# massquantity/tdfo

Measured on AMD Instinct MI355X. Metric: examples/sec (whole node) DLRM on Criteo-1TB-shaped synthetic, higher is better.
Workload: dtype bf16; 1 GPU; model=DLRM, global_batch=8192, parallelism=single-gpu, tables=criteo-1tb, embedding_dim=128, per_gpu_batch=8192

## Files before the change

### csrc/bindings.cpp

```cpp
#include <cmath>
#include <cstring>

#include <ATen/ATen.h>
#include <ATen/hip/HIPContext.h>
#include <torch/library.h>

#include "tdfo_kernels.h"

namespace {

using at::Tensor;

hipStream_t cur_stream() { return at::hip::getCurrentHIPStream().stream(); }

const uint16_t* bf16_ptr(const Tensor& t) {
  TORCH_CHECK(t.scalar_type() == at::kBFloat16, "expected bf16 tensor");
  return reinterpret_cast<const uint16_t*>(t.data_ptr());
}
uint16_t* bf16_mut(const Tensor& t) {
  TORCH_CHECK(t.scalar_type() == at::kBFloat16, "expected bf16 tensor");
  return reinterpret_cast<uint16_t*>(t.data_ptr());
}
void check_dev(const Tensor& t, const char* name) {
  TORCH_CHECK(t.is_cuda(), name, " must be a GPU tensor");
// ... 1087 lines not shown
  const float* bp[3] = {nullptr, nullptr, nullptr};
  int64_t bst[3] = {0, 0, 0};
  for (int i = 0; i < 3; ++i) {
    if (*bs[i]) {
      const Tensor& b = **bs[i];
      check_dev(b, "bias");
      TORCH_CHECK(b.scalar_type() == at::kFloat && b.dim() == 1 && b.size(0) >= nout[i],
                  "bottom_mlp_fwd: bias fp32 1-D");
      bp[i] = b.data_ptr<float>();
      bst[i] = b.stride(0);
    }
  }
  a.b0 = bp[0]; a.b1 = bp[1]; a.b2 = bp[2]; a.bs0 = bst[0]; a.bs1 = bst[1]; a.bs2 = bst[2];
  a.y0 = bf16_mut(y0); a.y1 = bf16_mut(y1); a.y2 = bf16_mut(y2);
  a.ldy0 = y0.stride(0); a.ldy1 = y1.stride(0); a.ldy2 = y2.stride(0);
  a.M = (int)M;
  if (dense) {
    check_dev(*dense, "dense");
    TORCH_CHECK(dense->scalar_type() == at::kFloat && dense->dim() == 2 && dense->size(0) == M &&
                dense->stride(1) == 1 && dense->size(1) <= 16 && dense->size(1) < x.size(1),
                "bottom_mlp_fwd: dense fp32 [M, nd < 16] rows");
    a.dense = dense->data_ptr<float>(); a.ld_dense = dense->stride(0);
    a.nd = (int)dense->size(1);
    a.x_out = bf16_mut(x);
    if (label_src) {
      TORCH_CHECK(label_dst && label_src->scalar_type() == at::kFloat &&
                  label_dst->scalar_type() == at::kFloat && label_src->is_contiguous() &&
                  label_dst->is_contiguous() && label_src->numel() >= M &&
                  label_dst->numel() >= M, "bottom_mlp_fwd: labels fp32 [M]");
      a.label_src = label_src->data_ptr<float>(); a.label_dst = label_dst->data_ptr<float>();
    }
  }
  tdfo::bottom_mlp_fwd(a, cur_stream());
}

void check_bf16_buf(const Tensor& t, int64_t n, const char* name) {
  check_dev(t, name);
  TORCH_CHECK(t.scalar_type() == at::kBFloat16 && t.is_contiguous() && t.numel() >= n, name,
              ": bf16 contiguous buffer too small");
}

void rw_rows_gather(const Tensor& Wt, const Tensor& recv, int64_t W, int64_t cap, const Tensor& out) {
  check_dev(Wt, "W");
  TORCH_CHECK(Wt.scalar_type() == at::kFloat && Wt.is_contiguous() && Wt.dim() == 2, "W fp32 2-D");
  TORCH_CHECK(Wt.size(0) <= (1LL << 32), "rw: owner rows must fit 32-bit row keys");
  const int64_t D = Wt.size(1);
  TORCH_CHECK(D == 16 || D == 32 || D == 64 || D == 128 || D == 256, "rw_rows_gather: D unsupported");
  check_i64(recv, "recv");
  TORCH_CHECK(recv.numel() == W * (cap + 1), "rw recv buffer must be [W][cap+1]");
  check_bf16_buf(out, W * (cap + 1) * D, "rw rows out");
  tdfo::rw_rows_gather(Wt.data_ptr<float>(), (int)D, recv.data_ptr<int64_t>(), (int)W, cap,
                       bf16_mut(out), cur_stream());
}

void rw_rows_scatter(const Tensor& send, int64_t W, int64_t cap, int64_t B, int64_t D,
                     const Tensor& rows, const Tensor& region, int64_t ld, const Tensor& map,
                     int64_t nrw) {
  check_i64(send, "send");
  TORCH_CHECK(send.numel() == W * (cap + 1), "rw send buffer must be [W][cap+1]");
  TORCH_CHECK(D == 16 || D == 32 || D == 64 || D == 128 || D == 256, "rw_rows_scatter: D unsupported");
  TORCH_CHECK(ld >= nrw * D && ld % 4 == 0, "rw_rows_scatter: row stride");
  TORCH_CHECK(B * ld < (1LL << 31), "rw_rows_scatter: region offsets must fit int32");
  check_bf16_buf(rows, W * (cap + 1) * D, "rw rows");
  check_bf16_buf(region, B * ld, "rw pooled region");
  check_dev(map, "rw map");
  TORCH_CHECK(map.scalar_type() == at::kInt && map.numel() >= W * (cap + 1), "rw map int32 [W][cap+1]");
// ... 873 lines not shown
  m.def("embedding_bwd(Tensor(a!) W, Tensor row_offset, Tensor indices, Tensor offsets, Tensor grad_off, "
        "Tensor? psw, int T, int B, bool mean, int key_bits, Tensor grad, int grad_stride, int opt, "
        "Tensor(b!)? state1, Tensor(c!)? state2, Tensor hyper, float eps, float beta1, float beta2, "
        "float weight_decay, Tensor(d!)? dense_grad, int segsort, int sr_seed=0, "
        "Tensor(e!)? sr_counter=None, bool sr=False) -> ()");
  m.def("embedding_bwd_workspace(int nnz, int D) -> int", [](int64_t nnz, int64_t D) {
    return (int64_t)tdfo::embedding_bwd_workspace(nnz < 1 ? 1 : nnz, (int)D);
  });
  m.def("embedding_bwd_prepare(Tensor W, Tensor row_offset, Tensor indices, Tensor offsets, "
        "Tensor grad_off, Tensor? psw, int T, int B, bool mean, int key_bits, int grad_stride, "
        "int segsort, Tensor(a!) workspace, Tensor? bag_len=None, Tensor(b!)? sr_counter=None) -> ()");
  m.def("embedding_bwd_apply(Tensor(a!) W, Tensor row_offset, Tensor indices, Tensor offsets, "
        "Tensor grad_off, Tensor? psw, int T, int B, bool mean, int key_bits, Tensor grad, "
        "int grad_stride, int opt, Tensor(b!)? state1, Tensor(c!)? state2, Tensor hyper, "
        "float eps, float beta1, float beta2, float weight_decay, Tensor(d!)? dense_grad, "
        "int segsort, Tensor(e!) workspace, int sr_seed=0, Tensor? sr_counter=None, "
        "bool sr=False) -> ()");
  m.def("embedding_dense_update(Tensor(a!) W, Tensor(d!) grad, int rows, int opt, Tensor(b!)? state1, "
        "Tensor(c!)? state2, Tensor hyper, float eps, float beta1, float beta2, "
        "float weight_decay, bool clear_grad) -> ()");
  m.def("rw_bucketize_workspace(int n, int W) -> int", rw_bucketize_workspace);
  m.def("rw_bucketize(Tensor ids, Tensor meta, int nrw, int W, int B, int cap, int n, "
        "Tensor(a!) send, Tensor(b!) workspace, Tensor(c!) overflow) -> ()");
  m.def("rw_pool(Tensor Wt, Tensor recv, Tensor meta, int nrw, int W, int B, int cap, bool mean, "
        "Tensor(a!) starts, Tensor(b!) out, int out_ld) -> ()");
  m.def("embedding_bwd_prepare_rw(Tensor W, Tensor recv, Tensor meta, int nrw, int Wsz, int B, "
        "int cap, bool mean, int key_bits, int grad_ld, int dummy_row, Tensor(a!) workspace, "
        "int rows=0) -> ()");
  m.def("rw_rows_gather(Tensor Wt, Tensor recv, int W, int cap, Tensor(a!) out) -> ()");
  m.def("bottom_mlp_fwd_ok(int k0, int n0, int n1, int n2) -> bool", bottom_mlp_fwd_ok);
  m.def("bottom_mlp_fwd(Tensor x, Tensor w0, Tensor w1, Tensor w2, Tensor? b0, Tensor? b1, "
        "Tensor? b2, Tensor(a!) y0, Tensor(b!) y1, Tensor(c!) y2, Tensor? dense, Tensor? label_src, "
        "Tensor(d!)? label_dst) -> ()");
  m.def("rw_rows_scatter(Tensor send, int W, int cap, int B, int D, Tensor rows, Tensor(a!) region, "
        "int ld, Tensor(b!) map, int nrw) -> ()");
  m.def("rw_grads_gather(Tensor map, int W, int cap, int D, Tensor dregion, Tensor(a!) gsend) -> ()");
  m.def("embedding_bwd_apply_rw(Tensor(a!) W, int Wsz, int B, int cap, bool mean, int key_bits, "
        "Tensor grad, int opt, Tensor(b!)? state1, Tensor(c!)? state2, Tensor hyper, float eps, "
        "float beta1, float beta2, float weight_decay, Tensor(d!) workspace) -> ()");
  m.def("dense_optimizer(Tensor(a!) p, Tensor g, Tensor(b!)? m, Tensor(c!)? v, Tensor(d!)? p_bf16, int opt, "
        "Tensor hyper, float beta1, float beta2, float eps, float wd, float momentum, Tensor? found_inf, "
        "Tensor[] seg_slabs, int[] seg_start, int[] seg_splits) -> ()");
  m.def("check_finite(Tensor g, Tensor(a!) found) -> ()");
  m.def("sort_pairs(Tensor keys, Tensor vals, int key_bits) -> (Tensor, Tensor)");
  m.def("cast_bf16(Tensor x, Tensor(a!) y) -> ()");
  m.def("bf16_stochastic_round(Tensor x, int seed, Tensor counter, int row0, Tensor(a!) out) -> ()");
  m.def("synth_criteo(int seed, int rank, int batch_index, int B, Tensor rows, Tensor pooling, "
        "Tensor base, int dist, float alpha, Tensor w_dense, Tensor table_bias, Tensor(a!) dense, "
        "Tensor(b!) ids, Tensor(c!) label) -> ()");
  m.def("synth_ids(int seed, int rank, int index_base, int B, Tensor rows, Tensor pooling, "
        "Tensor base, int dist, float alpha, Tensor counter, int nnz, Tensor(a!) ids) -> ()");
  m.def("synth_dense(int seed, int rank, int index_base, int B, Tensor rows, Tensor pooling, "
        "Tensor base, int dist, float alpha, Tensor counter, Tensor w_dense, Tensor table_bias, "
        "Tensor(a!) x0, Tensor(b!) label) -> ()");
  m.def("batch_load(Tensor dense, Tensor(a!) x0, Tensor ids, Tensor(b!) ids_dst, Tensor label, "
        "Tensor(c!) label_dst) -> ()");
  m.def("head_bce(Tensor H, Tensor w, Tensor b, Tensor label, float inv_n, bool relu_mask, "
        "Tensor(a!) logits, Tensor(b!) dH, Tensor(c!) part) -> ()");
  m.def("head_reduce(Tensor part, int nparts, int K, Tensor(a!) grad, Tensor(b!) loss_acc, "
        "Tensor(c!)[] bumps, bool defer) -> ()");
  m.def("reduce_rows(Tensor inp, int rows, int n, int ld, Tensor(a!) out, bool accumulate, float scale) -> ()");
  m.def("colsum(Tensor x, Tensor(a!) out, bool accumulate) -> ()");
  m.def("slab_reduce(Tensor[] slabs, int[] splits, Tensor(a!)[] outs) -> ()");
  m.def("seg_copy(Tensor src, Tensor(a!) dst, Tensor chunks, int src_n, int dst_n) -> ()");
  m.def("piece_copy(Tensor(a!) buf, Tensor pieces, int B, int w, int extent) -> ()");
  m.def("auc_hist(Tensor logits, Tensor labels, int nb, Tensor(a!) hist) -> ()");
// ... 23 lines not shown

TORCH_LIBRARY_IMPL(tdfo, CUDA, m) {
  m.impl("gemm", gemm);
  m.impl("attention_fwd", attention_fwd);
  m.impl("encoder_layer_fwd", encoder_layer_fwd);
  m.impl("encoder_layer_bwd", encoder_layer_bwd);
  m.impl("attention_bwd", attention_bwd);
  m.impl("attention_stream_fwd", attention_stream_fwd);
  m.impl("attention_stream_bwd", attention_stream_bwd);
  m.impl("layernorm_fwd", layernorm_fwd);
  m.impl("layernorm_bwd", layernorm_bwd);
  m.impl("seq_prologue_fwd", seq_prologue_fwd);
  m.impl("rank_metrics", rank_metrics);
  m.impl("topk_scores", topk_scores);
  m.impl("seq_prologue_bwd", seq_prologue_bwd);
  m.impl("gather_columns", gather_columns);
  m.impl("concat_features", concat_features);
  m.impl("batch_load", batch_load);
  m.impl("synth_criteo", synth_criteo);
  m.impl("split_features", split_features);
  m.impl("cross_bwd", cross_bwd);
  m.impl("interaction_fwd", interaction_fwd);
  m.impl("interaction_bwd", interaction_bwd);
  m.impl("embedding_bag_fwd", embedding_bag_fwd);
  m.impl("embedding_bwd", embedding_bwd);
  m.impl("embedding_bwd_prepare", embedding_bwd_prepare);
  m.impl("embedding_bwd_apply", embedding_bwd_apply);
  m.impl("embedding_dense_update", embedding_dense_update);
  m.impl("rw_bucketize", rw_bucketize);
  m.impl("rw_pool", rw_pool);
  m.impl("embedding_bwd_prepare_rw", embedding_bwd_prepare_rw);
  m.impl("rw_rows_gather", rw_rows_gather);
  m.impl("bottom_mlp_fwd", bottom_mlp_fwd);
  m.impl("rw_rows_scatter", rw_rows_scatter);
  m.impl("rw_grads_gather", rw_grads_gather);
  m.impl("embedding_bwd_apply_rw", embedding_bwd_apply_rw);
  m.impl("dense_optimizer", dense_optimizer);
  m.impl("check_finite", check_finite);
  m.impl("sort_pairs", sort_pairs);
  m.impl("cast_bf16", cast_bf16);
  m.impl("bf16_stochastic_round", bf16_stochastic_round);
  m.impl("slab_reduce", slab_reduce);
  m.impl("synth_ids", synth_ids);
  m.impl("synth_dense", synth_dense);
  m.impl("seg_copy", seg_copy);
  m.impl("piece_copy", piece_copy);
  m.impl("head_bce", head_bce);
  m.impl("reduce_rows", reduce_rows);
  m.impl("head_reduce", head_reduce);
  m.impl("colsum", colsum);
  m.impl("auc_hist", auc_hist);
  m.impl("two_tower", two_tower);
  m.impl("reduce_adam", reduce_adam);
  m.impl("linear_xent", linear_xent);
  m.impl("linear_xent_rows", linear_xent_rows);
  m.impl("linear_bce_rows", linear_bce_rows);
  m.impl("sample_ids", sample_ids);
  m.impl("jagged_to_dense", jagged_to_dense);
  m.impl("dense_to_jagged", dense_to_jagged);
  m.impl("jagged_ids_to_dense", jagged_ids_to_dense);
}

TORCH_LIBRARY_IMPL(tdfo, CPU, m) {
  m.impl("auc_hist", auc_hist);
}
```

### csrc/include/tdfo_kernels.h

```cpp
#pragma once
#include <hip/hip_runtime.h>
#include <stdint.h>

namespace tdfo {

struct GemmArgs {
  const uint16_t* A; int64_t lda; int a_col;
  const uint16_t* B; int64_t ldb; int b_col;
  int M, N, K, splits;
  const float* bias; int64_t bias_stride;
  int relu;
  const uint16_t* mask; int64_t ldm;
  uint16_t* C; int64_t ldc;
  float* C32; int64_t ldc32;
  const uint16_t* mul; int64_t ldmul;
  const uint16_t* add; int64_t ldadd;
  uint16_t* C2; int64_t ldc2;
  int csum_on, csum_col;
};
void gemm_bf16(const GemmArgs& a, hipStream_t s);


void gemm_group(const GemmArgs* a, int n, hipStream_t s);
int gemm_pairing(int v);
// ... 116 lines not shown

void embedding_dense_update(const EmbBwdArgs& a, int64_t rows, const float* grad, float* clear,
                            hipStream_t s);

struct SynthArgs {
  uint64_t seed; int rank; int64_t batch_index;
  int B, num_dense, T;
  const int64_t* rows; const int* pooling; const int64_t* base;
  int dist; double alpha;
  const float* w_dense; const float* table_bias;
  float* dense; int64_t* ids; float* label;
  const float* index_ptr; uint16_t* x0; int64_t ldx;
};
void synth_criteo(const SynthArgs& a, hipStream_t s);
void synth_ids(const SynthArgs& a, hipStream_t s);
void synth_dense(const SynthArgs& a, hipStream_t s);

struct BotMlpArgs {
  const uint16_t* x; int64_t ldx;
  const uint16_t* w0; const uint16_t* w1; const uint16_t* w2;
  int64_t ldw0, ldw1, ldw2;
  const float* b0; const float* b1; const float* b2;
  int64_t bs0, bs1, bs2;
  uint16_t* y0; uint16_t* y1; uint16_t* y2;
  int64_t ldy0, ldy1, ldy2;
  int M;
  const float* dense = nullptr; int64_t ld_dense = 0; int nd = 0;
  uint16_t* x_out = nullptr;
  const float* label_src = nullptr; float* label_dst = nullptr;
};
bool bottom_mlp_fwd_supported(int k0, int n0, int n1, int n2);
void bottom_mlp_fwd(const BotMlpArgs& a, hipStream_t s);

struct RwBucketArgs {
  const int64_t* ids; const int64_t* meta;
  int nrw, W, B; int64_t cap; int64_t n;
  int64_t* send; int32_t* overflow; int32_t* need;
};
size_t rw_bucketize_workspace(int64_t n, int W);
void rw_bucketize(const RwBucketArgs& a, void* ws, hipStream_t s);
struct RwPoolArgs {
  const float* Wt; int D; const int64_t* recv; const int64_t* meta;
  int nrw, W, B; int64_t cap; int mean;
  int32_t* starts; void* out; int out_f32; int64_t out_ld;
};
void rw_pool(const RwPoolArgs& a, hipStream_t s);
void rw_rows_gather(const float* Wt, int D, const int64_t* recv, int W, int64_t cap,
                    uint16_t* out, hipStream_t s);
void rw_rows_scatter(const int64_t* send, int W, int64_t cap, int B, int D, const uint16_t* rows,
                     uint16_t* region, int64_t ld, int32_t* map, hipStream_t s);
void rw_grads_gather(const int32_t* map, int W, int64_t cap, int D, const uint16_t* dregion,
                     uint16_t* gsend, hipStream_t s);
void embedding_bwd_prepare_rw(const EmbBwdArgs& a, const int64_t* recv, const int64_t* meta,
                              int nrw, int W, int64_t cap, int64_t grad_ld, int64_t dummy_row,
                              int rows, hipStream_t s);

enum DenseOpt { OPT_ADAMW = 0, OPT_ADAM = 1, OPT_SGD = 2, OPT_ADAGRAD = 3 };
struct DenseOptArgs {
  float* p; const float* g; float* m; float* v; uint16_t* p_bf16;
  int64_t n; int opt;
  const float* hyper;
  float beta1, beta2, eps, weight_decay, momentum;
  const float* found_inf;
  int nseg;
  int64_t seg_start[16], seg_len[16];
  int seg_splits[16];
// ... 216 lines not shown
```

### tdfo_amd/models/dlrm.py

```python
from __future__ import annotations

import math
import os
import warnings
from dataclasses import dataclass, field
from typing import List, Optional, Sequence

import torch

from ..utils.capture import graph_capture
from .. import ops
from .dlrm_dcn import DCNMixin
from .dlrm_streams import StreamGraphsMixin
from .dlrm_multirank import MultiRankStreamsMixin
from ..parallel.comm import as_comm, dense_comm_for
from ..sparse.planner import ShardingPlan, plan_sharding
from ..sparse.sharded import ShardedEmbeddingBags
from ..sparse.tables import EmbOptimConfig, TableConfig
from ..utils.flat import FlatParams

CRITEO_1TB_ROWS = [39884406, 39043, 17289, 7420, 20263, 3, 7120, 1543, 63, 38532951, 2953546,
                   403346, 10, 2208, 11938, 155, 4, 976, 14, 39979771, 25641295, 39664984, 585935,
                   12972, 108, 36]
CRITEO_KAGGLE_ROWS = [1460, 583, 10131227, 2202608, 305, 24, 12517, 633, 3, 93145, 5683, 8351593,
# ... 198 lines not shown
        opt = DENSE_OPTS[cfg.dense_opt]
        self.dense_opt = opt
        fp.finalize(dev, with_adam=opt in (ops.OPT_ADAMW, ops.OPT_ADAM))
        self.fp = fp
        self._ar_split = fp.offset(self.top_layers[0].name + ".w")
        self._init_dense()
        if world_size > 1:
            self.comm.broadcast(fp.p, src=0)
        fp.sync_bf16()
        self._defer_top_wgrad = (world_size > 1 if cfg.defer_wgrad is None
                                 else bool(cfg.defer_wgrad))
        bf = torch.bfloat16

        def z(*shape, dt=bf):
            return torch.zeros(*shape, dtype=dt, device=dev)

        def act_in(L: Lin):
            t = z(B, L.wcols)
            t[:, L.bcol] = 1.0
            return t

        self.x0 = act_in(self.bottom_layers[0])
        self.bot_in = [self.x0] + [act_in(L) for L in self.bottom_layers[1:]]
        self.h_out = z(B, D)
        Lb = self.bottom_layers
        self._fused_bottom = (
            dev.type == "cuda" and len(Lb) == 3 and D == Lb[2].out
            and os.environ.get("TDFO_FUSED_BOTTOM", "1") != "0"
            and Lb[0].in_k == Lb[0].wcols and not Lb[1].bias_in_k and not Lb[2].bias_in_k
            and Lb[1].in_k == Lb[0].out and Lb[2].in_k == Lb[1].out
            and ops.bottom_mlp_fwd_ok(Lb[0].in_k, Lb[0].out, Lb[1].out, Lb[2].out))
        self._bot_load_fold = os.environ.get("TDFO_BOT_LOAD_FOLD", "1") != "0"
        self._head_side = os.environ.get("TDFO_HEAD_SIDE", "1") != "0"
        self.bot_grad = [z(B, L.out) for L in self.bottom_layers]
        self.top_in = [act_in(L) for L in self.top_layers]
        self.t_out = z(B, self.head_k)
        self.top_grad = [z(B, L.out) for L in self.top_layers]
        self.dz = z(B, self.top_layers[0].in_k)
        self.label = z(B, dt=torch.float32)
        self.ids = torch.zeros(self.emb.nnz_local, dtype=torch.int64, device=dev)
        self.emb.bind_ids(self.ids)
        if cfg.interaction == "dcn":
            Lc, Wd, r = cfg.dcn_layers, self.top_real, cfg.dcn_rank
            self.dcn_x = [z(B, Wd) for _ in range(Lc)] + [self.top_in[0]]
            self.dcn_h = [act_in(u) for u in self.dcn_u]
            self.dcn_y = [z(B, Wd) for _ in range(Lc)]
            self.dcn_dx = [z(B, Wd) for _ in range(Lc + 1)]
            self.dcn_dx0acc = z(B, Wd)
            nb = Lc if self._defer_top_wgrad else 1
            self.dcn_dhl = [z(B, r) for _ in range(nb)]
            self.dcn_dyl = [z(B, Wd) for _ in range(nb)]
        self._x0_alias = False
        if (cfg.interaction == "dcn" and not self._defer_top_wgrad
                and self.emb.alias_pooled(self.dcn_x[0], self.dcn_dx[0], D)):
            self._x0_alias = True
            self.h_out = self.dcn_x[0][:, :D]
        self.logits = z(B, dt=torch.float32)
        self.nparts = ops.head_parts(B)
        self.head_part = z(self.nparts * (self.head_k + 2), dt=torch.float32)
        self.loss_sum = z(1, dt=torch.float32)
        self._pair_bwd = dev.type == "cuda"
        dcn = cfg.interaction == "dcn"
        if dev.type == "cuda" and not os.environ.get("TDFO_GEMM_POLICY"):
            ops.gemm_policy(5 if dcn else 0)
        self._gemm_pol = ops.gemm_policy(-1) if dev.type == "cuda" else None
        self._csum = not (dcn and dev.type == "cuda" and ops.gemm_policy(-1) in (4, 5))
# ... 133 lines not shown
        self._next = (dense, ids, label)
        self._primed = True
        self._mr_inflight = True

    def set_next_batch(self, dense: torch.Tensor, ids: torch.Tensor, label: torch.Tensor):
        if self.graph == "mstreams":
            self._mr_stage_next(dense, ids, label)
            return
        self._next = (dense, ids, label)

    def _m_load_next(self):
        if self._whole_capture:
            sx, si, sl = self._stg
            self.x0.copy_(sx)
            self.ids.copy_(si)
            self.label.copy_(sl)
            return
        dense, ids, label = self._next
        ops.batch_load(dense, self.x0, ids, self.ids, label, self.label)

    def _m_ids_exchange_next(self):
        self.emb.stage_fwd_ids_exchange(async_op=True, lagged=self._rw_lagged)

    def _rw_resolve(self):
        if self._rw_lagged and self.emb.rw_resolve_need():
            self.sync_streams()
            self.emb.rw_redo()

    def _fwd(self, L: Lin, x, out, relu=True):
        W = self.fp.bf16(L.name + ".w")
        bias = None if L.bias_in_k else self.fp.param(L.name + ".w")[:, L.bcol]
        ops.gemm(x[:, :L.in_k], False, W[:, :L.in_k], False, bias, relu, None, out, None, 1)

    def _bwd(self, L: Lin, x, dy, dx, x_is_relu, wgrad_now: bool = True):
        if not wgrad_now:
            self._dgrad(L, x, dy, dx, x_is_relu)
            return
        with ops.gemm_batch(self._pair_bwd and dx is not None):
            self._wgrad_gemm(L, x, dy)
            self._dgrad(L, x, dy, dx, x_is_relu)

    def _wg_splits(self, M: int, N: int) -> int:
        return ops.wgrad_splits(M, N, self.B, 256, slots=self._wg_slots)

    def _wgrad_n(self, L: Lin) -> int:
        return L.in_k if self._csum else L.wcols

    def _wgrad(self, L: Lin, x, dy):
        self._wgrad_gemm(L, x, dy)

    def _wgrad_gemm(self, L: Lin, x, dy):
        csum = -1 if (L.bias_in_k or not self._csum) else L.bcol
        n = self._wgrad_n(L)
        g = self.fp.grad(L.name + ".w").view(-1)
        if L.name in self.wslab:
            sl, S = self.wslab[L.name]
            ops.gemm(dy, True, x[:, :n], True, None, False, None, None, sl, S,
                     ldc32=L.wcols, csum_col=csum)
        else:
            ops.gemm(dy, True, x[:, :n], True, None, False, None, None, g, 1,
                     ldc32=L.wcols, csum_col=csum)
        return None

    def _dgrad(self, L: Lin, x, dy, dx, x_is_relu):
        if dx is not None:
            n = min(dx.shape[1], L.in_k)
            W = self.fp.bf16(L.name + ".w")
            ops.gemm(dy, False, W[:, :n], True, None, False,
                     x[:, :n] if x_is_relu else None, dx[:, :n], None, 1)

    def _stages(self):
# ... 129 lines not shown
        if self._pipe_lookup and self._ev_lookup is not None and self._side() is not None:
            torch.cuda.current_stream().wait_event(self._ev_lookup)
        self.emb.forward_wait()

    def _m_mark_loaded(self):
        if self._ev_loaded is not None and not self._whole_capture:
            self._ev_loaded.record(torch.cuda.current_stream())

    def _m_out_exchange_next(self):
        self.emb.stage_fwd_out_exchange()
        if self._ev_lookup is not None and not self._whole_capture:
            self._ev_lookup.record(torch.cuda.current_stream())

    def _s_top(self):
        self._s_top_a()
        self._s_top_b()

    def _s_top_a(self):
        cfg, fp, B = self.cfg, self.fp, self.B
        D, F = cfg.embedding_dim, self.F
        emb = self.emb
        if self._ps is not None and not self._mstream:
            self._wait(self._ps, torch.cuda.current_stream())
            with torch.cuda.stream(self._ps):
                emb.stage_bwd_prepare()
        h = self.h_out
        L0 = self.top_layers[0]
        if cfg.interaction == "dot":
            ops.interaction_fwd(h, emb.recv, self.slot_off, self.slot_stride, F, D, self.top_in[0],
                                L0.bcol)
        else:
            self._dcn_forward(h)
        n = len(self.top_layers)
        for i, L in enumerate(self.top_layers):
            out = self.top_in[i + 1][:, :L.out] if i + 1 < n else self.t_out
            self._fwd(L, self.top_in[i], out)
        K = self.head_k
        head = fp.param("head")
        ops.head_bce(self.t_out, head[:K], head[K:], self.label, 1.0 / (B * self.world), True,
                     self.logits, self.top_grad[-1], self.head_part)
        defer = self._head_side and self.device.type == "cuda"
        ops.head_reduce(self.head_part, self.nparts, K, fp.grad("head"), self.loss_sum,
                        (self.dense_hyper, self.emb_hyper), defer=defer)
        for i in reversed(range(n)):
            L = self.top_layers[i]
            if i > 0:
                dx = self.top_grad[i - 1]
            else:
                dx = self.dz if cfg.interaction == "dot" else self.dcn_dx[-1]
            self._bwd(L, self.top_in[i], self.top_grad[i], dx, x_is_relu=i > 0,
                      wgrad_now=not self._defer_top_wgrad)
            if defer:
                ops.flush_side_job()

    def _s_top_b(self):
        cfg = self.cfg
        D, F = cfg.embedding_dim, self.F
        emb = self.emb
        h = self.h_out
        if cfg.interaction == "dot":
            ops.interaction_bwd(self.dz, h, emb.recv, self.slot_off, self.slot_stride, F, D,
                                self.bot_grad[-1], emb.d_recv, self.slot_off, self.slot_stride,
                                True)
        else:
            self._dcn_backward(h)
        if not self._whole_capture:
            emb.stage_bwd_local(self.emb_hyper)
        if not self._mstream and self._ps is not None:
            self._wait(torch.cuda.current_stream(), self._ps)

    def _s_top_wgrad(self):
        if self._defer_top_wgrad:
            with ops.gemm_batch(self._pair_bwd):
                for i in reversed(range(len(self.top_layers))):
                    self._wgrad_gemm(self.top_layers[i], self.top_in[i], self.top_grad[i])
                for i in reversed(range(len(self.dcn_u))):
                    dy, _ = self._dcn_bufs(i)
                    self._wgrad_gemm(self.dcn_u[i], self.dcn_h[i], dy)
            for i in reversed(range(len(self.dcn_u))):
                self._dcn_wgrad_v(i)

    def _s_bottom_bwd(self):
        for i in reversed(range(len(self.bottom_layers))):
            L = self.bottom_layers[i]
            dx = self.bot_grad[i - 1] if i > 0 else None
            self._bwd(L, self.bot_in[i], self.bot_grad[i], dx, x_is_relu=i > 0)

    def _reduce_slabs(self, lo: int, hi: int):
        mine = [(sl, S, g) for off, sl, S, g in self._slab_sums if lo <= off < hi]
        if mine:
            ops.slab_reduce(mine)

    def _ar_issue(self, lo: int, hi: int):
        self._reduce_slabs(lo, hi)
        g = self.fp.g[lo:hi]
        if self.cfg.dense_comm == "bf16":
            if getattr(self, "_g16", None) is None:
                self._g16 = torch.empty(self.fp.g.numel(), dtype=torch.bfloat16,
                                        device=self.device)
            b = self._g16[lo:hi]
            ops.cast_bf16(g, b)
            return (self.dcomm.all_reduce(b, async_op=True), g, b)
        return (self.dcomm.all_reduce(g, async_op=True), None, None)

    def _m_allreduce_top_start(self):
        self._ar_top = None
        if self.world > 1:
            self._ar_top = self._ar_issue(self._ar_split, self.fp.g.numel())

    def _m_allreduce_start(self):
        self._ar_work = None
        if self.world > 1:
            self._ar_work = self._ar_issue(0, self._ar_split)

    def _s_emb_update(self):
        self.emb.stage_bwd_update(self.emb_hyper)

    def _m_allreduce_wait(self, names=("_ar_top", "_ar_work")):
# ... 232 lines not shown
```

### tdfo_amd/ops/__init__.py

```python
from __future__ import annotations

import os

import torch

from . import reference as ref
from ._ext import available as native_available
from ._ext import ops as _native
from .reference import (EMB_ADAGRAD, EMB_ADAM, EMB_DENSE_GRAD, EMB_ROWWISE_ADAGRAD,
                        EMB_SGD, OPT_ADAGRAD, OPT_ADAM, OPT_ADAMW, OPT_SGD, key_bits_for)


def _gpu(t: torch.Tensor) -> bool:
    return t.is_cuda


def bottom_mlp_fwd_ok(k0: int, n0: int, n1: int, n2: int) -> bool:
    return bool(native_available() and _native().bottom_mlp_fwd_ok(int(k0), int(n0), int(n1),
                                                                    int(n2)))


def bottom_mlp_fwd(x, w0, w1, w2, b0, b1, b2, y0, y1, y2, dense=None, label=None):
    ls, ld = label if label is not None else (None, None)
    _native().bottom_mlp_fwd(x, w0, w1, w2, b0, b1, b2, y0, y1, y2, dense, ls, ld)
# ... 369 lines not shown

def dense_optimizer(p, g, m, v, p_bf16, opt, hyper, beta1=0.9, beta2=0.999, eps=1e-8, wd=0.0,
                    momentum=0.0, found_inf=None, segments=()):
    if _gpu(p):
        _native().dense_optimizer(p, g, m, v, p_bf16, opt, hyper, beta1, beta2, eps, wd, momentum,
                                  found_inf, [s[1] for s in segments],
                                  [int(s[0]) for s in segments], [int(s[2]) for s in segments])
    else:
        if segments:
            g = g.clone()
            for start, slab, splits in segments:
                n = slab.numel() // splits
                g[start:start + n] = slab.view(splits, n).sum(0)
        ref.dense_optimizer(p, g, m, v, p_bf16, opt, hyper, beta1, beta2, eps, wd, momentum,
                            found_inf)


def check_finite(g, found):
    if _gpu(g):
        _native().check_finite(g, found)
    else:
        ref.check_finite(g, found)


def head_parts(B: int) -> int:
    return (B + 15) // 16


def head_bce(H, w, b, label, inv_n, relu_mask, logits, dH, part):
    if _gpu(H):
        _native().head_bce(H, w, b, label, inv_n, relu_mask, logits, dH, part)
    else:
        ref.head_bce(H, w, b, label, inv_n, relu_mask, logits, dH, part)


def reduce_rows(inp, rows, n, ld, out, accumulate=False, scale=1.0):
    if _gpu(inp):
        _native().reduce_rows(inp, rows, n, ld, out, accumulate, scale)
    else:
        ref.reduce_rows(inp, rows, n, ld, out, accumulate, scale)


class SegmentMap:

    CHUNK = 4096

    def __init__(self, pieces, device):
        self.device = torch.device(device)
        pieces = [(int(a), int(b), int(n)) for a, b, n in pieces if int(n) > 0]
        self.src_n = max([a + n for a, _, n in pieces], default=0)
        self.dst_n = max([b + n for _, b, n in pieces], default=0)
        self.n = sum(n for _, _, n in pieces)
        if self.device.type == "cuda":
            ch = []
            for a, b, n in pieces:
                for o in range(0, n, self.CHUNK):
                    ch.append((a + o, b + o, min(self.CHUNK, n - o)))
            self.chunks = torch.tensor(ch if ch else [[0, 0, 0]], dtype=torch.int64,
                                       device=self.device).view(-1, 3)
            self.nchunks = len(ch)
        else:
            idx = torch.zeros(self.dst_n, dtype=torch.int64)
            for a, b, n in pieces:
                idx[b:b + n] = torch.arange(a, a + n)
            self.index = idx

# ... 495 lines not shown
```

Measured before the change: 20.11 million examples/s.

## Fuse last top-MLP layer forward, BCE head, and dgrad into one kernel

Adds a fused HIP kernel that computes the last top-MLP layer (512->256 GEMM with bias+ReLU), the BCE head (logits, loss partials, head gradient), and the layer's input gradient (dgrad with ReLU mask) in one launch, keeping the activation tile in LDS. This removes separate GEMM, head_bce and dgrad launches and the HBM round trips of the intermediate activations. The layer's weight gradient is paired with the next layer's backward GEMM batch, or optionally with the bottom MLP. Cost: heavy LDS use limits occupancy, and the kernel only supports fixed dimensions.

```diff
diff --git a/csrc/bindings.cpp b/csrc/bindings.cpp
--- a/csrc/bindings.cpp
+++ b/csrc/bindings.cpp
@@ -1143,6 +1143,50 @@
     }
   }
   tdfo::bottom_mlp_fwd(a, cur_stream());
+}
+
+bool top_tail_ok(int64_t k, int64_t n, int64_t head_k) {
+  return tdfo::top_tail_supported((int)k, (int)n, (int)head_k);
+}
+
+void top_tail(const Tensor& x, const Tensor& w, const Tensor& bias, const Tensor& t,
+              const Tensor& hw, const Tensor& hb, const Tensor& label, double inv_n,
+              const Tensor& logits, const Tensor& dt, const Tensor& part, const Tensor& dx) {
+  TORCH_CHECK(!g_gemm_batch.on, "top_tail inside ops.gemm_batch");
+  const Tensor* ts[5] = {&x, &w, &t, &dt, &dx};
+  const char* nm[5] = {"x", "w", "t", "dt", "dx"};
+  for (int i = 0; i < 5; ++i) {
+    check_dev(*ts[i], nm[i]);
+    TORCH_CHECK(ts[i]->scalar_type() == at::kBFloat16 && ts[i]->dim() == 2 &&
+                ts[i]->stride(1) == 1 && ts[i]->stride(0) % 8 == 0 && aligned16(ts[i]->data_ptr()),
+                "top_tail: ", nm[i], " must be bf16 2-D, unit column stride, 16-B rows");
+  }
+  const int64_t B = x.size(0), K = x.size(1), N = w.size(0);
+  TORCH_CHECK(B >= 1 && B < (1LL << 31), "top_tail: batch");
+  TORCH_CHECK(tdfo::top_tail_supported((int)K, (int)N, (int)hw.numel()) && w.size(1) == K,
+              "top_tail: unsupported dims");
+  TORCH_CHECK(t.size(0) == B && t.size(1) == N && dt.size(0) == B && dt.size(1) == N &&
+              dx.size(0) == B && dx.size(1) == K, "top_tail: output shapes");
+  check_dev(bias, "bias");
+  TORCH_CHECK(bias.scalar_type() == at::kFloat && bias.dim() == 1 && bias.size(0) == N,
+              "top_tail: bias fp32 [N]");
+  check_f32c(hw, "head w"); check_f32c(hb, "head b"); check_f32c(label, "label");
+  check_f32c(logits, "logits"); check_f32c(part, "part");
+  TORCH_CHECK(hb.numel() == 1 && label.numel() == B && logits.numel() == B, "top_tail: head shapes");
+  TORCH_CHECK(part.numel() >= tdfo::head_bce_parts((int)B) * (N + 2), "top_tail: part too small");
+  tdfo::TopTailArgs a{};
+  a.x = bf16_ptr(x); a.ldx = x.stride(0);
+  a.w = bf16_ptr(w); a.ldw = w.stride(0);
+  a.bias = bias.data_ptr<float>(); a.bs = bias.stride(0);
+  a.t = bf16_mut(t); a.ldt = t.stride(0);
+  a.hw = hw.data_ptr<float>(); a.hb = hb.data_ptr<float>();
+  a.label = label.data_ptr<float>(); a.inv_n = (float)inv_n;
+  a.logits = logits.data_ptr<float>();
+  a.dt = bf16_mut(dt); a.lddt = dt.stride(0);
+  a.part = part.data_ptr<float>();
+  a.dx = bf16_mut(dx); a.lddx = dx.stride(0);
+  a.B = (int)B;
+  tdfo::top_tail(a, cur_stream());
 }
 
 void check_bf16_buf(const Tensor& t, int64_t n, const char* name) {
@@ -2082,6 +2126,10 @@
   m.def("bottom_mlp_fwd(Tensor x, Tensor w0, Tensor w1, Tensor w2, Tensor? b0, Tensor? b1, "
         "Tensor? b2, Tensor(a!) y0, Tensor(b!) y1, Tensor(c!) y2, Tensor? dense, Tensor? label_src, "
         "Tensor(d!)? label_dst) -> ()");
+  m.def("top_tail_ok(int k, int n, int head_k) -> bool", top_tail_ok);
+  m.def("top_tail(Tensor x, Tensor w, Tensor bias, Tensor(a!) t, Tensor hw, Tensor hb, "
+        "Tensor label, float inv_n, Tensor(b!) logits, Tensor(c!) dt, Tensor(d!) part, "
+        "Tensor(e!) dx) -> ()");
   m.def("rw_rows_scatter(Tensor send, int W, int cap, int B, int D, Tensor rows, Tensor(a!) region, "
         "int ld, Tensor(b!) map, int nrw) -> ()");
   m.def("rw_grads_gather(Tensor map, int W, int cap, int D, Tensor dregion, Tensor(a!) gsend) -> ()");
@@ -2171,6 +2219,7 @@
   m.impl("embedding_bwd_prepare_rw", embedding_bwd_prepare_rw);
   m.impl("rw_rows_gather", rw_rows_gather);
   m.impl("bottom_mlp_fwd", bottom_mlp_fwd);
+  m.impl("top_tail", top_tail);
   m.impl("rw_rows_scatter", rw_rows_scatter);
   m.impl("rw_grads_gather", rw_grads_gather);
   m.impl("embedding_bwd_apply_rw", embedding_bwd_apply_rw);
diff --git a/csrc/include/tdfo_kernels.h b/csrc/include/tdfo_kernels.h
--- a/csrc/include/tdfo_kernels.h
+++ b/csrc/include/tdfo_kernels.h
@@ -172,6 +172,22 @@
 bool bottom_mlp_fwd_supported(int k0, int n0, int n1, int n2);
 void bottom_mlp_fwd(const BotMlpArgs& a, hipStream_t s);
 
+struct TopTailArgs {
+  const uint16_t* x; int64_t ldx;
+  const uint16_t* w; int64_t ldw;
+  const float* bias; int64_t bs;
+  uint16_t* t; int64_t ldt;
+  const float* hw; const float* hb;
+  const float* label; float inv_n;
+  float* logits;
+  uint16_t* dt; int64_t lddt;
+  float* part;
+  uint16_t* dx; int64_t lddx;
+  int B;
+};
+bool top_tail_supported(int k, int n, int head_k);
+void top_tail(const TopTailArgs& a, hipStream_t s);
+
 struct RwBucketArgs {
   const int64_t* ids; const int64_t* meta;
   int nrw, W, B; int64_t cap; int64_t n;
diff --git a/csrc/kernels/top_tail.hip b/csrc/kernels/top_tail.hip
--- /dev/null
+++ b/csrc/kernels/top_tail.hip
@@ -0,0 +1,331 @@
+#include "tdfo_common.h"
+#include "tdfo_kernels.h"
+
+namespace tdfo {
+namespace {
+
+typedef __attribute__((ext_vector_type(4))) uint32_t u32x4;
+typedef __attribute__((ext_vector_type(2))) uint32_t u32x2;
+typedef __attribute__((address_space(1))) const void* gptr_t;
+
+constexpr int TM = 32, KX = 512, NT = 256, HK = 256;
+constexpr int SLOT = 64 * 1024;
+constexpr int R_W = 0, R_X = SLOT, R_T = 2 * SLOT, R_RED = R_T + TM * NT * 2;
+constexpr int RED_LD = HK + 2;
+constexpr int TAIL_LDS = R_RED + 2 * 4 * RED_LD * 4;
+static_assert(TAIL_LDS <= 160 * 1024, "LDS per workgroup");
+
+__device__ __forceinline__ int swz(int r, int c) { return r * 128 + ((c ^ (r & 7)) << 4); }
+
+__device__ __forceinline__ bf16x8_t frag(const TDFO_LDS char* img, int r0, int ks, int lane) {
+  const int r = r0 + (lane & 15);
+  return *(const TDFO_LDS bf16x8_t*)(img + swz(r, ks * 4 + (lane >> 4)));
+}
+
+__device__ __forceinline__ int t_off(int m, int n) {
+  return (n >> 6) * (TM * 128) + swz(m, (n & 63) >> 3) + (n & 7) * 2;
+}
+
+__device__ __forceinline__ bf16x8_t gfrag(const uint16_t* W, int64_t ldw, int r0, int kb,
+                                          int lane) {
+  const u32x4 v = *(const u32x4*)(W + (int64_t)(r0 + (lane & 15)) * ldw + kb + 8 * (lane >> 4));
+  return __builtin_bit_cast(bf16x8_t, v);
+}
+
+__device__ __forceinline__ int swz_col(int k) {
+  return ((k & 3) | (((k >> 3) & 1) << 2)) << 1;
+}
+
+__device__ __forceinline__ void glds16_asm(const void* src, TDFO_LDS char* dst) {
+  const uint32_t lds = __builtin_amdgcn_readfirstlane((uint32_t)(uintptr_t)dst);
+  asm volatile("s_mov_b32 m0, %1\n\tglobal_load_lds_dwordx4 %0, off"
+               :: "v"(src), "s"(lds) : "memory", "m0");
+}
+
+constexpr int W_PIECES = 16;
+
+__device__ __forceinline__ void stage_w(const uint16_t* W, int64_t ldw, int kt,
+                                        TDFO_LDS char* slot, int w, int lane) {
+  TDFO_LDS char* img = slot + w * (64 * 256);
+#pragma unroll
+  for (int ii = 0; ii < W_PIECES; ++ii) {
+    const int kr = ii * 4 + (lane >> 4);
+    const int c = (lane & 15) ^ swz_col(kr);
+    glds16_asm(W + (int64_t)(kt * 64 + kr) * ldw + w * 128 + c * 8, img + ii * 1024);
+  }
+}
+
+__device__ __forceinline__ bf16x8_t frag_col(const TDFO_LDS char* tile, int c0, int ks,
+                                             int lane) {
+  const int i = lane & 15, g = lane >> 4;
+  const int q = i >> 2, p = i & 3;
+  const int m = c0 + 4 * p;
+  s16x4_t v[2];
+#pragma unroll
+  for (int h = 0; h < 2; ++h) {
+    const int k = ks * 32 + 8 * g + 4 * h + q;
+    const int off = k * 256 + (((m >> 3) ^ swz_col(k)) << 4) + ((m & 7) << 1);
+    v[h] = __builtin_amdgcn_ds_read_tr16_b64_v4i16((TDFO_LDS s16x4_t*)(tile + off));
+  }
+  s16x8_t r = {v[0][0], v[0][1], v[0][2], v[0][3], v[1][0], v[1][1], v[1][2], v[1][3]};
+  return __builtin_bit_cast(bf16x8_t, r);
+}
+
+__device__ __forceinline__ void lds_wait() { asm volatile("s_waitcnt lgkmcnt(0)" ::: "memory"); }
+
+__device__ __forceinline__ void raw_barrier() {
+  __builtin_amdgcn_sched_barrier(0);
+  __builtin_amdgcn_s_barrier();
+  asm volatile("" ::: "memory");
+  __builtin_amdgcn_sched_barrier(0);
+}
+
+__device__ __forceinline__ float head_sample(const float (&hv)[4], const float (&wr)[4],
+                                             float hbias, float y, float inv_n, bool lane0,
+                                             float& x, float (&dw)[4], float& db, float& lsum) {
+#pragma clang fp contract(off)
+  float d = 0.f;
+#pragma unroll
+  for (int u = 0; u < 4; ++u) d = __builtin_fmaf(hv[u], wr[u], d);
+  x = wave_sum(d) + hbias;
+  const float sig = 1.f / (1.f + __expf(-x));
+  const float g = (sig - y) * inv_n;
+  if (lane0) {
+    lsum += __builtin_fmaf(-y, x, fmaxf(x, 0.f)) + log1pf(__expf(-fabsf(x)));
+    db += g;
+  }
+#pragma unroll
+  for (int u = 0; u < 4; ++u) dw[u] = __builtin_fmaf(g, hv[u], dw[u]);
+  return g;
+}
+
+__global__ __launch_bounds__(256) void top_tail_kernel(TopTailArgs a) {
+  extern __shared__ __attribute__((aligned(16))) char smem_raw[];
+  TDFO_LDS char* sm = (TDFO_LDS char*)smem_raw;
+  const int tid = threadIdx.x, lane = tid & 63;
+  const int w = __builtin_amdgcn_readfirstlane(tid >> 6);
+  const int m0 = blockIdx.x * TM;
+  const int B = a.B;
+
+  constexpr int J = NT / 64, S = KX / 32, PD = 8;
+  const int c0 = w * (NT / 4);
+  u32x4 xv[KX / 64];
+  {
+    const int r = tid >> 3, c = tid & 7;
+    int gr = m0 + r;
+    gr = gr < B ? gr : B - 1;
+#pragma unroll
+    for (int kt = 0; kt < KX / 64; ++kt)
+      xv[kt] = *(const u32x4*)(a.x + (int64_t)gr * a.ldx + kt * 64 + c * 8);
+  }
+  bf16x8_t b[S][J];
+#pragma unroll
+  for (int s = 0; s < PD; ++s)
+#pragma unroll
+    for (int j = 0; j < J; ++j) b[s][j] = gfrag(a.w, a.ldw, c0 + 16 * j, 32 * s, lane);
+  float bv[J][4];
+#pragma unroll
+  for (int j = 0; j < J; ++j)
+#pragma unroll
+    for (int r = 0; r < 4; ++r)
+      bv[j][r] = a.bias[(int64_t)(c0 + 16 * j + 4 * (lane >> 4) + r) * a.bs];
+  const int e0 = lane * 4;
+  float wr[4];
+#pragma unroll
+  for (int u = 0; u < 4; ++u) wr[u] = a.hw[e0 + u];
+  const float hbias = a.hb[0];
+  float yv[2][4];
+#pragma unroll
+  for (int g = 0; g < 2; ++g)
+#pragma unroll
+    for (int q = 0; q < 4; ++q) yv[g][q] = a.label[min(m0 + 16 * g + w + 4 * q, B - 1)];
+  {
+    const int r = tid >> 3, c = tid & 7;
+#pragma unroll
+    for (int kt = 0; kt < KX / 64; ++kt)
+      *(TDFO_LDS u32x4*)(sm + R_X + kt * (TM * 128) + swz(r, c)) = xv[kt];
+  }
+  __syncthreads();
+  {
+    f32x4_t acc[2][J];
+#pragma unroll
+    for (int i = 0; i < 2; ++i)
+#pragma unroll
+      for (int j = 0; j < J; ++j) acc[i][j] = (f32x4_t){0.f, 0.f, 0.f, 0.f};
+#pragma unroll
+    for (int s = 0; s < S; ++s) {
+      if (s + PD < S) {
+#pragma unroll
+        for (int j = 0; j < J; ++j)
+          b[s + PD][j] = gfrag(a.w, a.ldw, c0 + 16 * j, 32 * (s + PD), lane);
+      }
+      bf16x8_t af[2];
+#pragma unroll
+      for (int i = 0; i < 2; ++i)
+        af[i] = frag(sm + R_X + (s >> 1) * (TM * 128), 16 * i, s & 1, lane);
+#pragma unroll
+      for (int i = 0; i < 2; ++i)
+#pragma unroll
+        for (int j = 0; j < J; ++j)
+          acc[i][j] = __builtin_amdgcn_mfma_f32_16x16x32_bf16(b[s][j], af[i], acc[i][j], 0, 0, 0);
+    }
+    stage_w(a.w, a.ldw, 0, sm + R_W, w, lane);
+#pragma unroll
+    for (int j = 0; j < J; ++j) {
+      const int n = c0 + 16 * j + 4 * (lane >> 4);
+#pragma unroll
+      for (int i = 0; i < 2; ++i) {
+        const int m = 16 * i + (lane & 15);
+        float v[4];
+#pragma unroll
+        for (int r = 0; r < 4; ++r) v[r] = fmaxf(acc[i][j][r] + bv[j][r], 0.f);
+        const u32x2 pk = {pack2bf(v[0], v[1]), pack2bf(v[2], v[3])};
+        if (m0 + m < B) *(u32x2*)(a.t + (int64_t)(m0 + m) * a.ldt + n) = pk;
+        *(TDFO_LDS u32x2*)(sm + R_T + t_off(m, n)) = pk;
+      }
+    }
+  }
+  __syncthreads();
+  stage_w(a.w, a.ldw, 1, sm + R_X, w, lane);
+
+  float* red = (float*)(smem_raw + R_RED);
+#pragma unroll
+  for (int g = 0; g < 2; ++g) {
+    const int s0 = m0 + 16 * g;
+    float dw[4] = {0.f, 0.f, 0.f, 0.f};
+    float db = 0.f, lsum = 0.f;
+    float hv[4][4];
+#pragma unroll
+    for (int q = 0; q < 4; ++q) {
+      const u32x2 tv = *(const TDFO_LDS u32x2*)(sm + R_T + t_off(16 * g + w + 4 * q, e0));
+      hv[q][0] = bf2f((uint16_t)(tv.x & 0xffff));
+      hv[q][1] = bf2f((uint16_t)(tv.x >> 16));
+      hv[q][2] = bf2f((uint16_t)(tv.y & 0xffff));
+      hv[q][3] = bf2f((uint16_t)(tv.y >> 16));
+    }
+#pragma unroll
+    for (int q = 0; q < 4; ++q) {
+      const int s = s0 + w + 4 * q;
+      if (s >= B) break;
+      float x;
+      const float gq = head_sample(hv[q], wr, hbias, yv[g][q], a.inv_n, lane == 0, x, dw, db, lsum);
+      if (lane == 0) a.logits[s] = x;
+      uint16_t hb16[4];
+#pragma unroll
+      for (int u = 0; u < 4; ++u) {
+        float gh = gq * wr[u];
+        if (!(hv[q][u] > 0.f)) gh = 0.f;
+        hb16[u] = f2bf(gh);
+      }
+      const u32x2 pk = {(uint32_t)hb16[0] | ((uint32_t)hb16[1] << 16),
+                        (uint32_t)hb16[2] | ((uint32_t)hb16[3] << 16)};
+      *(u32x2*)(a.dt + (int64_t)s * a.lddt + e0) = pk;
+      *(TDFO_LDS u32x2*)(sm + R_T + t_off(16 * g + w + 4 * q, e0)) = pk;
+    }
+    float* rw = red + (g * 4 + w) * RED_LD;
+#pragma unroll
+    for (int u = 0; u < 4; ++u) rw[e0 + u] = dw[u];
+    if (lane == 0) { rw[HK] = db; rw[HK + 1] = lsum; }
+  }
+  __syncthreads();
+#pragma unroll
+  for (int g = 0; g < 2; ++g) {
+    if (m0 + 16 * g < B) {
+      const float* rg = red + g * 4 * RED_LD;
+      for (int j = tid; j < RED_LD; j += 256)
+        a.part[(int64_t)(blockIdx.x * 2 + g) * RED_LD + j] =
+            rg[j] + rg[RED_LD + j] + rg[2 * RED_LD + j] + rg[3 * RED_LD + j];
+    }
+  }
+
+  constexpr int NJ = 8;
+  const TDFO_LDS char* wimg0 = sm + R_W + w * (64 * 256);
+  const TDFO_LDS char* wimg1 = sm + R_X + w * (64 * 256);
+  f32x4_t acc[2][NJ];
+#pragma unroll
+  for (int i = 0; i < 2; ++i)
+#pragma unroll
+    for (int j = 0; j < NJ; ++j) acc[i][j] = (f32x4_t){0.f, 0.f, 0.f, 0.f};
+  auto tile = [&](int kt, const TDFO_LDS char* wimg) {
+#pragma unroll
+    for (int ks = 0; ks < 2; ++ks) {
+      bf16x8_t af[2], bfr[NJ];
+#pragma unroll
+      for (int j = 0; j < NJ; ++j) bfr[j] = frag_col(wimg, 16 * j, ks, lane);
+#pragma unroll
+      for (int i = 0; i < 2; ++i) af[i] = frag(sm + R_T + kt * (TM * 128), 16 * i, ks, lane);
+#pragma unroll
+      for (int i = 0; i < 2; ++i)
+#pragma unroll
+        for (int j = 0; j < NJ; ++j)
+          acc[i][j] = __builtin_amdgcn_mfma_f32_16x16x32_bf16(bfr[j], af[i], acc[i][j], 0, 0, 0);
+    }
+  };
+  asm volatile("s_waitcnt vmcnt(0) lgkmcnt(0)" ::: "memory");
+  raw_barrier();
+  tile(0, wimg0);
+  lds_wait();
+  raw_barrier();
+  stage_w(a.w, a.ldw, 2, sm + R_W, w, lane);
+  tile(1, wimg1);
+  lds_wait();
+  raw_barrier();
+  stage_w(a.w, a.ldw, 3, sm + R_X, w, lane);
+  asm volatile("s_waitcnt vmcnt(%0)" :: "i"(W_PIECES) : "memory");
+  raw_barrier();
+  const int rho = lane & 15, gq = lane >> 4;
+  const int mrow = (gq & 1) * 16 + rho;
+  const int ncol = w * 128 + 8 * (gq >> 1);
+  u32x4 mk[NJ];
+  {
+    int gr = m0 + mrow;
+    gr = gr < B ? gr : B - 1;
+#pragma unroll
+    for (int j = 0; j < NJ; ++j)
+      mk[j] = *(const u32x4*)(a.x + (int64_t)gr * a.ldx + ncol + 16 * j);
+  }
+  tile(2, wimg0);
+  asm volatile("s_waitcnt vmcnt(0)" ::: "memory");
+  raw_barrier();
+  tile(3, wimg1);
+#pragma unroll
+  for (int j = 0; j < NJ; ++j) {
+    float v[8];
+#pragma unroll
+    for (int r = 0; r < 4; ++r) {
+      const float p = acc[0][j][r] + 0.f, q = acc[1][j][r] + 0.f;
+      const auto sw = __builtin_amdgcn_permlane16_swap(__float_as_uint(p), __float_as_uint(q),
+                                                       false, false);
+      v[r] = __uint_as_float(sw[0]);
+      v[4 + r] = __uint_as_float(sw[1]);
+    }
+    const uint32_t mu[4] = {mk[j].x, mk[j].y, mk[j].z, mk[j].w};
+#pragma unroll
+    for (int q = 0; q < 4; ++q) {
+      if (!(bf2f((uint16_t)(mu[q] & 0xffff)) > 0.f)) v[2 * q] = 0.f;
+      if (!(bf2f((uint16_t)(mu[q] >> 16)) > 0.f)) v[2 * q + 1] = 0.f;
+    }
+    if (m0 + mrow < B)
+      *(u32x4*)(a.dx + (int64_t)(m0 + mrow) * a.lddx + ncol + 16 * j) =
+          u32x4{pack2bf(v[0], v[1]), pack2bf(v[2], v[3]), pack2bf(v[4], v[5]),
+                pack2bf(v[6], v[7])};
+  }
+}
+
+}
+
+bool top_tail_supported(int k, int n, int head_k) { return k == KX && n == NT && head_k == HK; }
+
+void top_tail(const TopTailArgs& a, hipStream_t s) {
+  if (a.B <= 0) return;
+  static bool attr = false;
+  if (!attr) {
+    TDFO_CHECK_HIP(hipFuncSetAttribute((const void*)top_tail_kernel,
+                                       hipFuncAttributeMaxDynamicSharedMemorySize, TAIL_LDS));
+    attr = true;
+  }
+  hipLaunchKernelGGL(top_tail_kernel, dim3((a.B + TM - 1) / TM), dim3(256), TAIL_LDS, s, a);
+  TDFO_CHECK_HIP(hipGetLastError());
+}
+
+}
diff --git a/tdfo_amd/models/dlrm.py b/tdfo_amd/models/dlrm.py
--- a/tdfo_amd/models/dlrm.py
+++ b/tdfo_amd/models/dlrm.py
@@ -254,6 +254,15 @@
             and ops.bottom_mlp_fwd_ok(Lb[0].in_k, Lb[0].out, Lb[1].out, Lb[2].out))
         self._bot_load_fold = os.environ.get("TDFO_BOT_LOAD_FOLD", "1") != "0"
         self._head_side = os.environ.get("TDFO_HEAD_SIDE", "1") != "0"
+        Lt = self.top_layers
+        self._top_tail = (
+            dev.type == "cuda" and len(Lt) >= 2 and not Lt[-1].bias_in_k
+            and Lt[-1].in_k == Lt[-2].out
+            and os.environ.get("TDFO_TOP_TAIL", "1") != "0"
+            and ops.top_tail_ok(Lt[-1].in_k, Lt[-1].out, self.head_k))
+        self._tail_wgrad_late = (world_size == 1 and not self._defer_top_wgrad
+                                 and cfg.opt_placement == "one_pass"
+                                 and os.environ.get("TDFO_TAIL_WGRAD", "top") == "bottom")
         self.bot_grad = [z(B, L.out) for L in self.bottom_layers]
         self.top_in = [act_in(L) for L in self.top_layers]
         self.t_out = z(B, self.head_k)
@@ -453,11 +462,13 @@
         bias = None if L.bias_in_k else self.fp.param(L.name + ".w")[:, L.bcol]
         ops.gemm(x[:, :L.in_k], False, W[:, :L.in_k], False, bias, relu, None, out, None, 1)
 
-    def _bwd(self, L: Lin, x, dy, dx, x_is_relu, wgrad_now: bool = True):
+    def _bwd(self, L: Lin, x, dy, dx, x_is_relu, wgrad_now: bool = True, also=None):
         if not wgrad_now:
             self._dgrad(L, x, dy, dx, x_is_relu)
             return
         with ops.gemm_batch(self._pair_bwd and dx is not None):
+            if also is not None:
+                self._wgrad_gemm(*also)
             self._wgrad_gemm(L, x, dy)
             self._dgrad(L, x, dy, dx, x_is_relu)
 
@@ -653,24 +664,38 @@
         else:
             self._dcn_forward(h)
         n = len(self.top_layers)
-        for i, L in enumerate(self.top_layers):
-            out = self.top_in[i + 1][:, :L.out] if i + 1 < n else self.t_out
-            self._fwd(L, self.top_in[i], out)
+        tail = self._top_tail
+        for i, L in enumerate(self.top_layers[:n - 1]):
+            self._fwd(L, self.top_in[i], self.top_in[i + 1][:, :L.out])
         K = self.head_k
         head = fp.param("head")
-        ops.head_bce(self.t_out, head[:K], head[K:], self.label, 1.0 / (B * self.world), True,
-                     self.logits, self.top_grad[-1], self.head_part)
+        if tail:
+            Lt = self.top_layers[-1]
+            ops.top_tail(self.top_in[-1][:, :Lt.in_k], fp.bf16(Lt.name + ".w")[:, :Lt.in_k],
+                         fp.param(Lt.name + ".w")[:, Lt.bcol], self.t_out, head[:K], head[K:],
+                         self.label, 1.0 / (B * self.world), self.logits, self.top_grad[-1],
+                         self.head_part, self.top_grad[-2][:, :Lt.in_k])
+        else:
+            self._fwd(self.top_layers[-1], self.top_in[-1], self.t_out)
+            ops.head_bce(self.t_out, head[:K], head[K:], self.label, 1.0 / (B * self.world),
+                         True, self.logits, self.top_grad[-1], self.head_part)
         defer = self._head_side and self.device.type == "cuda"
         ops.head_reduce(self.head_part, self.nparts, K, fp.grad("head"), self.loss_sum,
                         (self.dense_hyper, self.emb_hyper), defer=defer)
+        also = None
         for i in reversed(range(n)):
             L = self.top_layers[i]
+            if tail and i == n - 1:
+                if not self._defer_top_wgrad and not self._tail_wgrad_late:
+                    also = (L, self.top_in[i], self.top_grad[i])
+                continue
             if i > 0:
                 dx = self.top_grad[i - 1]
             else:
                 dx = self.dz if cfg.interaction == "dot" else self.dcn_dx[-1]
             self._bwd(L, self.top_in[i], self.top_grad[i], dx, x_is_relu=i > 0,
-                      wgrad_now=not self._defer_top_wgrad)
+                      wgrad_now=not self._defer_top_wgrad, also=also)
+            also = None
             if defer:
                 ops.flush_side_job()
 
@@ -705,6 +730,12 @@
         for i in reversed(range(len(self.bottom_layers))):
             L = self.bottom_layers[i]
             dx = self.bot_grad[i - 1] if i > 0 else None
+            if i == 0 and self._top_tail and self._tail_wgrad_late:
+                Lt = self.top_layers[-1]
+                with ops.gemm_batch(self._pair_bwd):
+                    self._wgrad_gemm(Lt, self.top_in[-1], self.top_grad[-1])
+                    self._wgrad_gemm(L, self.bot_in[0], self.bot_grad[0])
+                continue
             self._bwd(L, self.bot_in[i], self.bot_grad[i], dx, x_is_relu=i > 0)
 
     def _reduce_slabs(self, lo: int, hi: int):
diff --git a/tdfo_amd/ops/__init__.py b/tdfo_amd/ops/__init__.py
--- a/tdfo_amd/ops/__init__.py
+++ b/tdfo_amd/ops/__init__.py
@@ -425,6 +425,19 @@
         _native().head_bce(H, w, b, label, inv_n, relu_mask, logits, dH, part)
     else:
         ref.head_bce(H, w, b, label, inv_n, relu_mask, logits, dH, part)
+
+
+def top_tail_ok(k: int, n: int, head_k: int) -> bool:
+    return bool(native_available() and _native().top_tail_ok(int(k), int(n), int(head_k)))
+
+
+def top_tail(x, w, bias, t, hw, hb, label, inv_n, logits, dt, part, dx):
+    if _gpu(x):
+        _native().top_tail(x, w, bias, t, hw, hb, label, inv_n, logits, dt, part, dx)
+    else:
+        ref.gemm(x, False, w, False, bias, True, None, t, None, 1, None, None, None, 0, -1)
+        ref.head_bce(t, hw, hb, label, inv_n, True, logits, dt, part)
+        ref.gemm(dt, False, w, True, None, False, x, dx, None, 1, None, None, None, 0, -1)
 
 
 def reduce_rows(inp, rows, n, ld, out, accumulate=False, scale=1.0):
```

Result: slower. 19.81 million examples/s (-1.5%).
